# cfframe/spatial-VAE

Measured on AMD Instinct MI355X. Metric: images/sec (ELBO fwd+bwd+step), MNIST 28x28 batch=256, 1/2/4/8 GPU, higher is better.
Workload: dtype f32; 1 GPU; mnist-rotated-translated 28x28 z=2 H=500x2 tanh B=256 (BASELINE configs[1]); global_batch=256, per_gpu_batch=256, pixels=784, parallelism=dp1

## Files before the change

spatial_vae_amd/csrc/api.hip:

```cpp
#include <stdarg.h>
#include <stdio.h>
#include <stdlib.h>
#include <string.h>
#include <math.h>
#include <atomic>
#include <mutex>
#include <iterator>
#include <type_traits>
#include <unordered_map>
#include <vector>

#include "common.h"
#include <hip/hip_ext.h>
#include "dense.h"
#include "wgrad2.h"
#include "elementwise.h"
#include "encoder.h"
#include "split.h"

using namespace svae;

namespace {

thread_local char g_err[512] = "";
// ... 77 lines not shown
bool split_wgrad_on() {
    static const bool on = [] { const char* e = getenv("SVAE_SPLIT_WGRAD"); return !(e && e[0] == '0'); }();
    return on;
}

bool split_a0_fragments_only(const Geo& g) {
    static const bool on = [] { const char* e = getenv("SVAE_SPLIT_A0"); return e && e[0] == '1'; }();
    const char* fuse = getenv("SVAE_FUSE_OUT");
    return on && split_mode() && split_l0_on() && split_wgrad_on() && !(fuse && fuse[0] == '1') &&
           (g.act == SVAE_ACT_TANH || g.act == SVAE_ACT_SIGMOID) && g.ntile % 2 == 0 && g.L == 2 && g.in_dim == 2 &&
           !(g.flags & SVAE_FLAG_RESID);
}

int fuse_out_mode() {
    const char* e = getenv("SVAE_FUSE_OUT");
    if (!e) return 2;
    return e[0] == '0' ? 0 : (e[0] == '1' ? 1 : 2);
}
bool split_active(const Geo& g) {
    return split_mode() && (g.act == SVAE_ACT_TANH || g.act == SVAE_ACT_SIGMOID) && g.ntile % 2 == 0;
}
bool rank1_out(const Geo& g) {
    return fuse_out_mode() == 2 && !split_active(g) && g.C == 1 && g.L >= 2 && !(g.flags & SVAE_FLAG_RESID) &&
           (g.act == SVAE_ACT_TANH || g.act == SVAE_ACT_SIGMOID);
}

struct PlanBits {
    unsigned bits;
    unsigned long long seq;
};
std::mutex g_plan_mu;
std::unordered_map<const void*, PlanBits> g_plans;
unsigned long long g_plan_seq = 0;
unsigned plan_bits(const Geo& g) {
    return (rank1_out(g) ? 1u : 0u) | (split_active(g) ? 2u : 0u) | ((unsigned)fuse_out_mode() << 2) |
           (split_a0_fragments_only(g) ? 16u : 0u) | ((split_mode() && split_l0_on()) ? 32u : 0u);
}
void remember_plan(const void* saved, unsigned bits) {
    std::lock_guard<std::mutex> lk(g_plan_mu);
    if (g_plans.size() >= 4096) {
        const unsigned long long cut = g_plan_seq - 2048;
        for (auto it = g_plans.begin(); it != g_plans.end();) it = it->second.seq < cut ? g_plans.erase(it) : std::next(it);
    }
    g_plans[saved] = PlanBits{bits, g_plan_seq++};
}
long recorded_plan(const void* saved) {
    std::lock_guard<std::mutex> lk(g_plan_mu);
    auto it = g_plans.find(saved);
    return it == g_plans.end() ? -1L : (long)it->second.bits;
}

constexpr int kFinishMaxChunks = 64;
int finish_chunks(int N) {
    int c = (N + 1023) / 1024;
    return c < 1 ? 1 : (c > kFinishMaxChunks ? kFinishMaxChunks : c);
}

Plan make_plan(const Geo& g, void* saved, void* ws) {
    Plan p;
    const size_t MH = (size_t)g.Mp * g.Hp;
    Carver cs(saved);
    for (int l = 0; l < g.L; ++l) p.act[l] = cs.take<float>(MH);
    p.savedC = split_mode() ? cs.take<uint4>(MH / 4) : nullptr;
    float* swf[SVAE_MAX_HIDDEN];
    float* swb[SVAE_MAX_HIDDEN];
    for (int l = 0; l + 1 < g.L; ++l) {
        swf[l] = cs.take<float>((size_t)g.Hp * g.Hp);
        swb[l] = cs.take<float>((size_t)g.Hp * g.Hp);
    }
// ... 417 lines not shown
                               g.Hp, (const float*)pl.gscale);
        if (!aprev_cols)
            hipLaunchKernelGGL(split_cols_kernel, dim3(blocks_for(g.noct * g.Hp)), dim3(256), 0, st, aprev, pl.splitC[1],
                               g.noct, g.Hp, (const float*)nullptr);
    }
    Scope prof(K_WGRAD, st);
    static bool attr_set = false;
    if (!attr_set) {
        (void)hipFuncSetAttribute(reinterpret_cast<const void*>(&split_wgrad_kernel<true>),
                                  hipFuncAttributeMaxDynamicSharedMemorySize, kSplitWgradLds);
        (void)hipFuncSetAttribute(reinterpret_cast<const void*>(&split_wgrad_kernel<false>),
                                  hipFuncAttributeMaxDynamicSharedMemorySize, kSplitWgradLds);
        attr_set = true;
    }
    SplitWgradArgs w;
    w.dh = pl.splitC[0]; w.ap = aprev_cols ? aprev_cols : pl.splitC[1]; w.slab = pl.slab; w.bslab = pl.bslab; w.gscale = pl.gscale;
    w.nsteps = (long)g.Mp / 16; w.Hp = g.Hp; w.nblk1 = pl.wg_nblk1; w.S = pl.wg_S;
    const dim3 grid(pl.wg_nblk1 * pl.wg_nblk1 * pl.wg_S);
    if (cols_ready) hipLaunchKernelGGL(split_wgrad_kernel<false>, grid, dim3(256), kSplitWgradLds, st, w);
    else hipLaunchKernelGGL(split_wgrad_kernel<true>, grid, dim3(256), kSplitWgradLds, st, w);
}

int use_dense4(const Geo& g, int resid, int lastd) {
    const char* e = getenv("SVAE_DENSE4");
    const int mode = e ? (e[0] == '0' ? 0 : (e[0] == '2' ? 2 : 1)) : 3;
    if (mode == 0 || g.tiles % 4 != 0 || resid || lastd == 1) return 0;
    const bool nt2_ok = g.ntile % 2 == 0;
    if (mode == 2) return nt2_ok ? 2 : 1;
    if (mode == 1) return 1;
    const long wgs2 = ((g.tiles / 4 + 3) / 4) * (g.ntile / 2);
    return (nt2_ok && wgs2 >= 2048) ? 2 : 1;
}

template <int NT, bool DGRAD, bool FIRST, int LASTD, int CF>
void launch_dense4_v(const DenseArgs& a, long groups, long set0, long nsets, hipStream_t st) {
    const dim3 grid((unsigned)(((nsets + 7) / 8) * 8 * ((a.Hp / 32) / NT)));
    constexpr int lds = DenseCfg<NT>::LDS_BYTES + (FIRST ? 4 * 3 * 128 * 4 : 0);
    const long gend = (set0 + nsets) * 4 < groups ? (set0 + nsets) * 4 : groups;
    launch_gemm(dense4_kernel<NT, DGRAD, FIRST, LASTD, CF>, grid, dim3(256), (unsigned)lds, st, a, gend, set0);
}

struct DenseBlocks {
    int nt;
    long m_split;
    int nt_tail;
};

long dense4_main_sets(const Geo& g, long sets, bool tail_ok) {
    const char* e = getenv("SVAE_DENSE4_TAIL");
    if ((e && e[0] == '0') || !tail_ok) return sets;
    if (e && e[0] == '=') {
        const long k = atol(e + 1);
        return (k > 0 && k < sets) ? k : sets;
    }
    static const long slots = [] {
        int dev = 0, cus = 256;
        if (hipGetDevice(&dev) == hipSuccess) (void)hipDeviceGetAttribute(&cus, hipDeviceAttributeMultiprocessorCount, dev);
        return (long)cus * 2;
    }();
    const long nblk = g.ntile / 2;
    const long W = sets * nblk;
    if (slots % nblk != 0) return sets;
    const long full = (W / slots) * slots, rest = W - full;
    if (full < 2 * slots || rest == 0 || W >= 16 * slots || 20 * rest > 9 * slots) return sets;
    return full / nblk;
}

template <bool DGRAD, bool FIRST, int LASTD, int CF>
void launch_dense4_dual(const DenseArgs& a, long groups, long sets, long main_sets, hipStream_t st) {
    const unsigned ntile = (unsigned)(a.Hp / 32);
    const unsigned grid_main = (unsigned)(((main_sets + 7) / 8) * 8) * (ntile / 2);
    const unsigned grid_tail = (unsigned)(((sets - main_sets + 7) / 8) * 8) * ntile;
    constexpr int lds = DenseCfg<2>::LDS_BYTES + (FIRST ? 4 * 3 * 128 * 4 : 0);
    launch_gemm(dense4_dual_kernel<DGRAD, FIRST, LASTD, CF>, dim3(grid_main + grid_tail), dim3(256), (unsigned)lds, st, a, groups,
                main_sets, grid_main);
}

template <bool DGRAD>
DenseBlocks launch_dense(const Geo& g, const DenseArgs& a, hipStream_t st, bool first = false, int lastd = 0, int cf = 0) {
    took(DGRAD ? P_DENSE_FP32_DGRAD : P_DENSE_FP32_FWD);
    if (lastd) took(lastd == 1 ? P_OUT_BWD_FUSED_GENERIC : P_OUT_BWD_RANK1);
    Scope prof(DGRAD ? K_DENSE_DGRAD : K_DENSE_FWD, st, true);
    if (const int nt4 = use_dense4(g, a.resid, lastd)) {
        took(P_DENSE4);
        if (!DGRAD && cf > 0) took(P_DENSE4_CF);
        if (nt4 == 2) took(P_DENSE4_NT2);
        const long groups = g.tiles / 4;
        const long sets = (groups + 3) / 4;
        auto go = [&](auto nt_tag, long set0, long nsets) {
            constexpr int NT = decltype(nt_tag)::value;
            if constexpr (!DGRAD) {
                switch (cf) {
                    case 0: launch_dense4_v<NT, false, false, 0, 0>(a, groups, set0, nsets, st); break;
                    case 1: launch_dense4_v<NT, false, false, 0, 1>(a, groups, set0, nsets, st); break;
                    case 2: launch_dense4_v<NT, false, false, 0, 2>(a, groups, set0, nsets, st); break;
                    case 3: launch_dense4_v<NT, false, false, 0, 3>(a, groups, set0, nsets, st); break;
                    default: launch_dense4_v<NT, false, false, 0, 4>(a, groups, set0, nsets, st); break;
                }
            } else {
                if (first) {
                    if (lastd == 2) launch_dense4_v<NT, true, true, 2, 0>(a, groups, set0, nsets, st);
                    else if (lastd == 3) launch_dense4_v<NT, true, true, 3, 0>(a, groups, set0, nsets, st);
                    else launch_dense4_v<NT, true, true, 0, 0>(a, groups, set0, nsets, st);
                } else {
                    if (lastd == 2) launch_dense4_v<NT, true, false, 2, 0>(a, groups, set0, nsets, st);
                    else if (lastd == 3) launch_dense4_v<NT, true, false, 3, 0>(a, groups, set0, nsets, st);
                    else launch_dense4_v<NT, true, false, 0, 0>(a, groups, set0, nsets, st);
                }
            }
        };
        if (nt4 == 1) {
            go(std::integral_constant<int, 1>(), 0, sets);
            return DenseBlocks{1, (long)g.Mp, 1};
        }
        if (cf > 2) {
            if constexpr (!DGRAD) {
                if (cf == 3) launch_dense4_v<2, false, false, 0, 3>(a, groups, 0, sets, st);
                else launch_dense4_v<2, false, false, 0, 4>(a, groups, 0, sets, st);
            }
            return DenseBlocks{2, (long)g.Mp, 1};
        }
        const long main_sets = dense4_main_sets(g, sets, true);
        took(P_DENSE4_DUAL);
        if (main_sets < sets) took(P_DENSE4_TAIL);
        if constexpr (!DGRAD) {
            switch (cf) {
                case 0: launch_dense4_dual<false, false, 0, 0>(a, groups, sets, main_sets, st); break;
                case 1: launch_dense4_dual<false, false, 0, 1>(a, groups, sets, main_sets, st); break;
                default: launch_dense4_dual<false, false, 0, 2>(a, groups, sets, main_sets, st); break;
            }
        } else {
            if (first) {
                if (lastd == 2) launch_dense4_dual<true, true, 2, 0>(a, groups, sets, main_sets, st);
                else if (lastd == 3) launch_dense4_dual<true, true, 3, 0>(a, groups, sets, main_sets, st);
                else launch_dense4_dual<true, true, 0, 0>(a, groups, sets, main_sets, st);
            } else {
                if (lastd == 2) launch_dense4_dual<true, false, 2, 0>(a, groups, sets, main_sets, st);
                else if (lastd == 3) launch_dense4_dual<true, false, 3, 0>(a, groups, sets, main_sets, st);
                else launch_dense4_dual<true, false, 0, 0>(a, groups, sets, main_sets, st);
            }
        }
        return DenseBlocks{2, main_sets < sets ? main_sets * 512 : (long)g.Mp, 1};
    }
    const int nt = (first || lastd || cf) ? dense_nt_first(g.ntile) : dense_nt_for(g.ntile);
    static const bool xcd_grid = [] { const char* e = getenv("SVAE_XCD_GRID"); return !(e && e[0] == '0'); }();
    const long groups = (g.tiles + 3) / 4;
    const dim3 grid = (xcd_grid && g.ntile / nt > 1) ? dim3((unsigned)(((groups + 7) / 8) * 8 * (g.ntile / nt)))
                                                     : dim3((unsigned)groups, (unsigned)(g.ntile / nt));
    switch (nt) {
        case 16: launch_dense_nt<16, DGRAD>(a, grid, st, first, lastd, cf); break;
        case 8: launch_dense_nt<8, DGRAD>(a, grid, st, first, lastd, cf); break;
        case 4: launch_dense_nt<4, DGRAD>(a, grid, st, first, lastd, cf); break;
        case 2: launch_dense_nt<2, DGRAD>(a, grid, st, first, lastd, cf); break;
        default: launch_dense_nt<1, DGRAD>(a, grid, st, first, lastd, cf); break;
    }
    return DenseBlocks{nt, (long)g.Mp, nt};
}

template <int CL, int R1 = 0>
void launch_wgrad_c(const WgradArgs& w, dim3 grid, hipStream_t st) {
    static bool attr_set = false;
    if (!attr_set) {
        (void)hipFuncSetAttribute(reinterpret_cast<const void*>(&wgrad_kernel<CL, R1>), hipFuncAttributeMaxDynamicSharedMemorySize,
                                  kWgradLdsBytes);
        attr_set = true;
    }
    launch_gemm(wgrad_kernel<CL, R1>, grid, dim3(256), (unsigned)kWgradLdsBytes, st, w);
}

bool tail_merge_on() {
    const char* e = getenv("SVAE_TAIL_MERGE");
    return !(e && e[0] == '0');
}

bool use_wgrad2(int cl, int r1) {
// ... 39 lines not shown
template <int ACT>
void launch_layer0_fwd(const Geo& g, const Plan& pl, const PoseArgs& pa, float* a0, hipStream_t st) {
    Scope prof(K_LAYER0_FWD, st);
    const int oimg = g.Npad / 8;
    const int cpi = (oimg + kL0Chunk - 1) / kL0Chunk;
    const int opc = (oimg + cpi - 1) / cpi;
    const long nchunks = (long)g.B * cpi;
    const unsigned gy = (unsigned)(nchunks < 32768 ? nchunks : 32768);
    const unsigned gz = (unsigned)((nchunks + gy - 1) / gy);
    hipLaunchKernelGGL((layer0_fwd_kernel<ACT>), dim3(blocks_for(g.Hp * 2), gy, gz), dim3(256), 0, st, pa, pl.posebuf,
                       pl.tab, a0, row_geo(g), opc, (oimg + opc - 1) / opc, nchunks);
}

template <int ACT>
void launch_layer0_fwd_split(const Geo& g, const Plan& pl, const PoseArgs& pa, float* a0, bool saved_ok, hipStream_t st) {
    Scope prof(K_LAYER0_FWD, st);
    hipLaunchKernelGGL((layer0_fwd_split_kernel<ACT>), dim3((unsigned)g.tiles, (unsigned)(g.Hp / 64)), dim3(256), 0, st, pa,
                       pl.posebuf, pl.tab, split_a0_fragments_only(g) ? (float*)nullptr : a0, pl.splitA,
                       (saved_ok && g.L == 2) ? pl.savedC : (uint4*)nullptr, row_geo(g));
}

template <int C>
void launch_out_fwd(const Geo& g, const float* a, const svae_params* p, float* y, float* logits, hipStream_t st) {
    Scope prof(K_OUT_FWD, st);
    long nb = (g.noct + 3) / 4;
    if (nb > 4096) nb = 4096;
    hipLaunchKernelGGL((out_fwd_kernel<C>), dim3((unsigned)nb), dim3(256), 0, st, a, p->out_w, p->out_b, y, logits,
                       row_geo(g), g.H, (g.flags & SVAE_FLAG_SOFTPLUS) ? 1 : 0, g.noct);
}

template <int ACT, int C>
void launch_out_bwd_ac(const Geo& g, const Plan& pl, const float* a, const svae_params* p, float* dh, hipStream_t st) {
    Scope prof(K_OUT_BWD, st);
    hipLaunchKernelGGL((out_bwd_kernel<ACT, C>), dim3(blocks_for(g.Hp * 2), pl.ob_chunks), dim3(256), 0, st, a, pl.do_p,
                       p->out_w, dh, pl.wpart, pl.bpart, g.H, g.Hp, (long)g.Mp, g.noct, pl.ob_oct_per_chunk);
}
template <int ACT>
void launch_out_bwd_a(const Geo& g, const Plan& pl, const float* a, const svae_params* p, float* dh, hipStream_t st) {
    took(P_OUT_BWD_STREAM);
    switch (g.C) {
        case 1: launch_out_bwd_ac<ACT, 1>(g, pl, a, p, dh, st); break;
        case 2: launch_out_bwd_ac<ACT, 2>(g, pl, a, p, dh, st); break;
        case 3: launch_out_bwd_ac<ACT, 3>(g, pl, a, p, dh, st); break;
        default: launch_out_bwd_ac<ACT, 4>(g, pl, a, p, dh, st); break;
    }
}

}

extern "C" {

int svae_abi_version(void) { return SVAE_ABI_VERSION; }
const char* svae_last_error(void) { return g_err; }

size_t svae_saved_bytes(const svae_desc* d) {
    if (check_desc(d) != SVAE_OK) return 0;
    return make_plan(make_geo(*d), nullptr, nullptr).saved_bytes;
}

size_t svae_workspace_bytes(const svae_desc* d) {
    if (check_desc(d) != SVAE_OK) return 0;
    return make_plan(make_geo(*d), nullptr, nullptr).ws_bytes;
}

}

namespace {
int decoder_forward_impl(const svae_desc* d, const svae_params* p, const svae_pose* pose, const float* z, float* y,
// ... 99 lines not shown
}
}

extern "C" {

int svae_decoder_forward(const svae_desc* d, const svae_params* p, const svae_pose* pose, const float* z, float* y,
                         float* logits, void* saved, void* ws, size_t ws_bytes, svae_stream_t stream) {
    return decoder_forward_impl(d, p, pose, z, y, logits, saved, ws, ws_bytes, stream, nullptr, nullptr, nullptr);
}

int svae_decoder_forward_bce(const svae_desc* d, const svae_params* p, const svae_pose* pose, const float* z,
                             const float* target, float* y, float* logits, float* loglik, float* dll_dy, void* saved, void* ws,
                             size_t ws_bytes, svae_stream_t stream) {
    if (!target) return fail(SVAE_E_INVALID, "svae_decoder_forward_bce: target is null");
    return decoder_forward_impl(d, p, pose, z, y, logits, saved, ws, ws_bytes, stream, target, loglik, dll_dy);
}

int svae_decoder_backward(const svae_desc* d, const svae_params* p, const svae_pose* pose, const float* z,
                          const float* logits, const float* dy, const float* dy_scale, const void* saved,
                          const svae_grads* grads, float* dz, const svae_pose_grads* pg, void* ws, size_t ws_bytes,
                          svae_stream_t stream) {
    int rc;
    if ((rc = check_desc(d)) || (rc = check_params(d, p)) || (rc = check_pose(pose))) return rc;
    if (!logits || !dy || !saved || !grads) return fail(SVAE_E_INVALID, "logits, dy, saved and grads are required");
    if (d->Zd > 0 && !z) return fail(SVAE_E_INVALID, "latent_dim > 0 but z is null");
    if (reinterpret_cast<uintptr_t>(saved) & 255) return fail(SVAE_E_WORKSPACE, "saved not 256-byte aligned");
    if (pg && (pg->dtheta || pg->ddx) && pose->coords)
        return fail(SVAE_E_INVALID, "dtheta/ddx requested but the pose was given as explicit coords");
    const Geo g = make_geo(*d);
    {
        const long rec = recorded_plan(saved);
        if (rec >= 0 && (unsigned)rec != plan_bits(g))
            return fail(SVAE_E_INVALID, "svae_decoder_backward: `saved` was written by a forward call planned differently (plan "
                        "bits %ld then, %u now): the GEMM mode (svae_gemm_mode_set / SVAE_GEMM) or SVAE_FUSE_OUT changed between "
                        "the forward call and its backward call", rec, plan_bits(g));
    }
    const Plan pl = make_plan(g, const_cast<void*>(saved), ws);
    if ((rc = check_ws(pl, ws, ws_bytes))) return rc;
    hipStream_t st = static_cast<hipStream_t>(stream);
    const PoseArgs pa = pose_args(pose);
    const int resid = (g.flags & SVAE_FLAG_RESID) ? 1 : 0;
    const int fmode = fuse_out_mode();
    const bool split_bwd = split_active(g) && g.L >= 2 && fmode != 1;
    const bool r1 = rank1_out(g);

    {
        Scope prof(K_DLOGITS, st);
        if (split_bwd && hipMemsetAsync(pl.amax, 0, sizeof(unsigned), st) != hipSuccess) return fail(SVAE_E_LAUNCH, "memset failed");
        hipLaunchKernelGGL(dlogits_kernel, dim3(blocks_for((long)g.C * g.Mp)), dim3(256), 0, st, logits, dy, dy_scale,
                           pl.do_p, g.B, g.N, g.Npad, g.C, (g.flags & SVAE_FLAG_SOFTPLUS) ? 1 : 0, (long)g.Mp,
                           split_bwd ? pl.amax : (unsigned*)nullptr);
        if (split_bwd)
            hipLaunchKernelGGL(split_scale_kernel, dim3(1), dim3(256), 0, st, pl.amax, p->out_w, g.C, g.H, pl.gscale);
    }

    int cur = 0;
    const bool fused_out = r1 || (fmode == 1 && g.L >= 2 && !resid && (grads->hidden_w[g.L - 2] || grads->hidden_b[g.L - 2]));
    int ob_nparts = 0;
    static const bool ob_env = [] { const char* e = getenv("SVAE_SPLIT_OB"); return !(e && e[0] == '0'); }();
    const bool split_ob = ob_env && split_bwd && split_wgrad_on() && (grads->hidden_w[g.L - 2] || grads->hidden_b[g.L - 2]);
    if (split_ob) {
        const float* alast = pl.act[g.L - 1];
        float* dh32 = resid ? pl.dh[cur] : nullptr;
        const int nparts = g.act == SVAE_ACT_TANH ? launch_out_bwd_split_a<SVAE_ACT_TANH>(g, pl, alast, p, dh32, st)
                                                  : launch_out_bwd_split_a<SVAE_ACT_SIGMOID>(g, pl, alast, p, dh32, st);
        ob_nparts = nparts;
        Scope prof(K_SMALL_BWD, st);
        hipLaunchKernelGGL(out_bwd_reduce_kernel, dim3(g.C * ((g.Hp + 63) / 64) + 1), dim3(1024), 0, st, pl.wpart, pl.bpart,
// ... 406 lines not shown
```

spatial_vae_amd/csrc/dense.h:

```cpp
#pragma once
#include "common.h"

namespace svae {

struct DenseArgs {
    const float* in;
    const float* wp;
    float* out;
    const float* bias;
    const float* aux;
    long tiles;
    int Hp;
    int H;
    int act;
    int resid;
    PoseArgs pose;
    const float4* posebuf;
    const float* tab;
    float* sgtile;
    float* dfpart;
    long Mp;
    int N, Timg;
    const float* do_p;
    const float* out_w;
    int C;
    float* lpart;
};

template <int ACT, bool DGRAD>
__device__ __forceinline__ float4 dense_epilogue(float4 v, float bias, float4 aux) {
    if (DGRAD) {
        v.x *= act_grad<ACT>(aux.x); v.y *= act_grad<ACT>(aux.y);
        v.z *= act_grad<ACT>(aux.z); v.w *= act_grad<ACT>(aux.w);
    } else {
        v.x = act_fwd<ACT>(v.x + bias); v.y = act_fwd<ACT>(v.y + bias);
        v.z = act_fwd<ACT>(v.z + bias); v.w = act_fwd<ACT>(v.w + bias);
    }
    return v;
}

__device__ __forceinline__ void glds16(const float* gsrc, unsigned lds_byte_addr) {
    unsigned keep;
    asm volatile(
        "s_mov_b32 %0, m0\n\ts_mov_b32 m0, %2\n\ts_nop 0\n\tglobal_load_lds_dwordx4 %1, off\n\ts_mov_b32 m0, %0"
        : "=&s"(keep)
        : "v"(gsrc), "s"(lds_byte_addr)
        : "memory");
}
__device__ __forceinline__ void dma_wait_all() { asm volatile("s_waitcnt vmcnt(0)" ::: "memory"); }
__device__ __forceinline__ void glds16_s(const void* sbase, unsigned voff, unsigned lds_byte_addr) {
    unsigned keep;
    asm volatile(
        "s_mov_b32 %0, m0\n\ts_mov_b32 m0, %3\n\ts_nop 0\n\tglobal_load_lds_dwordx4 %1, %2\n\ts_mov_b32 m0, %0"
        : "=&s"(keep)
        : "v"(voff), "s"(sbase), "s"(lds_byte_addr)
        : "memory");
}

__device__ __forceinline__ void load_a_chunk(const float* p, float (&v)[4][4]) {
// ... 739 lines not shown
```

spatial_vae_amd/csrc/dense4.h:

```cpp
#pragma once
#include "dense.h"

namespace svae {

typedef float f32x4v __attribute__((ext_vector_type(4)));
typedef float f32x2v __attribute__((ext_vector_type(2)));

template <int OFF>
__device__ __forceinline__ void load_a4(const float* p, f32x4v& v) {
    asm volatile("global_load_dwordx4 %0, %1, off offset:%2" : "+v"(v) : "v"(p), "i"(OFF) : "memory");
}
template <int N>
__device__ __forceinline__ void wait_vm4(f32x4v& v) {
    asm volatile("s_waitcnt vmcnt(%1)" : "+v"(v) : "i"(N) : "memory");
}
template <int LASTD>
__device__ __forceinline__ f32x4v rank1_actgrad(f32x4v x) {
    f32x4v r;
#pragma unroll
    for (int i = 0; i < 4; ++i) r[i] = __builtin_fmaf(-x[i], x[i], LASTD == 2 ? 1.0f : x[i]);
    return r;
}

template <int NT>
struct Dense4Occ {
    static constexpr int value = NT == 1 ? 3 : 2;
};

template <int NT, bool DGRAD, bool FIRST, int LASTD, int CF>
__device__ __forceinline__ void dense4_body(const DenseArgs& a, long groups, long set0, unsigned bid) {
    static_assert(NT == 1 || NT == 2, "4 NT accumulator tiles: two waves per SIMD up to NT = 2");
    static_assert(!FIRST || DGRAD, "FIRST is a data-gradient epilogue");
    static_assert(LASTD == 0 || ((LASTD == 2 || LASTD == 3) && DGRAD), "LASTD: the rank-1 data-gradient forms only");
    static_assert(CF == 0 || (!DGRAD && CF <= SVAE_MAX_OUT), "CF = output channels of the forward epilogue's W_o contraction");
    extern __shared__ __attribute__((aligned(16))) float smem[];
    using Cfg = DenseCfg<NT>;
    constexpr int NB = Cfg::NB, G = Cfg::G, CHUNK = Cfg::CHUNK, NINSTR = Cfg::NINSTR;
    const int lane = threadIdx.x & 63;
    const int wave = __builtin_amdgcn_readfirstlane(threadIdx.x >> 6);
    const int nl = lane & 31, h = lane >> 5;
    const int Hp = a.Hp;
    const int noct = Hp / 8;
    const int nchunk = noct / G;
    const int ntile = Hp / 32;
    const int nblk = ntile / NT;
    const long local = bid >> 3;
    const int nb = (int)(local % nblk);
    const long set = set0 + (local / nblk) * 8 + (bid & 7);
    const long rg = set * 4 + wave;
    const bool live = rg < groups;
    const long rgl = live ? rg : groups - 1;

    const float* arow = a.in + ((rgl * 16 + (nl >> 1)) * (long)Hp + 4 * h) * 8 + (nl & 1) * 4;
    const float* bfrag = smem + lane * 4;
    const unsigned lds_base = (unsigned)(size_t)(__attribute__((address_space(3))) float*)smem;

    f32x16 acc[4][NT];
#pragma unroll
    for (int c = 0; c < 4; ++c)
#pragma unroll
        for (int t = 0; t < NT; ++t)
#pragma unroll
            for (int r = 0; r < 16; ++r) acc[c][t][r] = 0.0f;

    constexpr int PW = (NINSTR + 3) / 4;
    unsigned poff[PW], pm0[PW];
#pragma unroll
    for (int j = 0; j < PW; ++j) {
        const int idx = wave + 4 * j;
        const int gl = (idx < NINSTR ? idx : NINSTR - 1) / NT, tt = (idx < NINSTR ? idx : NINSTR - 1) % NT;
        poff[j] = (unsigned)(((gl * ntile + nb * NT + tt) * 256 + lane * 4) * 4);
        pm0[j] = lds_base + (unsigned)(idx < NINSTR ? idx : NINSTR - 1) * 1024u;
    }
    const unsigned chunk_bytes = (unsigned)(G * ntile) * 1024u;
    auto stage_piece = [&](int c, int buf, int j) {
        glds16_s(reinterpret_cast<const char*>(a.wp) + (long)c * chunk_bytes, poff[j], pm0[j] + (unsigned)(buf * CHUNK) * 4u);
    };
    auto stage = [&](int c, int buf) {
#pragma unroll
        for (int j = 0; j < PW; ++j) stage_piece(c, buf, j);
    };
    auto read_b = [&](int o, float4 (&b)[NT]) {
        const float* base = bfrag + ((o / G) & 1) * CHUNK + (o % G) * NT * 256;
#pragma unroll
        for (int t = 0; t < NT; ++t) b[t] = *reinterpret_cast<const float4*>(base + t * 256);
    };
    constexpr int P = PW;
    constexpr int PE = (P + 3) / 4;
    static_assert(G == 4, "the slot offsets assume 4 octets per chunk");

    float* rowx = smem + 2 * CHUNK + wave * (3 * 128);
    if (FIRST) {
#pragma unroll
        for (int rr = 0; rr < 2; ++rr) {
            const int row = lane + 64 * rr;
            const long tile = rgl * 4 + (row >> 5);
            const int b = (int)(tile / a.Timg);
            const int i = (int)(tile % a.Timg) * 32 + (row & 31);
            const float4 pb = a.posebuf[b];
            const float* cbase = a.pose.coords ? a.pose.coords + (long)b * a.N * 2 : a.pose.grid;
            const float2 g2 = *reinterpret_cast<const float2*>(cbase + (long)(i < a.N ? i : a.N - 1) * 2);
            const bool in = i < a.N;
            rowx[row] = in ? pb.x * g2.x - pb.y * g2.y + pb.z : 0.0f;
            rowx[128 + row] = in ? pb.y * g2.x + pb.x * g2.y + pb.w : 0.0f;
            if (LASTD != 0) rowx[256 + row] = a.do_p[rgl * 128 + row];
        }
    }
    stage(0, 0);
    stage(nchunk > 1 ? 1 : 0, 1);
    f32x4v av[G][4];
    float4 b0[NT], b1[NT];
#pragma unroll
    for (int gl = 0; gl < G; ++gl)
#pragma unroll
        for (int e = 0; e < 4; ++e) av[gl][e] = f32x4v{0.0f, 0.0f, 0.0f, 0.0f};
    load_a4<0>(arow, av[0][0]); load_a4<32>(arow, av[0][1]); load_a4<64>(arow, av[0][2]); load_a4<96>(arow, av[0][3]);
    load_a4<256>(arow, av[1][0]); load_a4<288>(arow, av[1][1]); load_a4<320>(arow, av[1][2]); load_a4<352>(arow, av[1][3]);
    load_a4<512>(arow, av[2][0]); load_a4<544>(arow, av[2][1]); load_a4<576>(arow, av[2][2]); load_a4<608>(arow, av[2][3]);
    load_a4<768>(arow, av[3][0]); load_a4<800>(arow, av[3][1]); load_a4<832>(arow, av[3][2]); load_a4<864>(arow, av[3][3]);
#pragma unroll
    for (int gl = 0; gl < G; ++gl)
#pragma unroll
        for (int e = 0; e < 4; ++e) wait_vm4<0>(av[gl][e]);
    __syncthreads();
    read_b(0, b0);
    const int spare = nchunk & 1;
    auto kstep = [&](const f32x4v& x, const float4 (&bf)[NT], int e) {
#pragma unroll
        for (int t = 0; t < NT; ++t) {
            const float bv = e == 0 ? bf[t].x : e == 1 ? bf[t].y : e == 2 ? bf[t].z : bf[t].w;
            acc[0][t] = __builtin_amdgcn_mfma_f32_32x32x2f32(x[0], bv, acc[0][t], 0, 0, 0);
            acc[1][t] = __builtin_amdgcn_mfma_f32_32x32x2f32(x[1], bv, acc[1][t], 0, 0, 0);
            acc[2][t] = __builtin_amdgcn_mfma_f32_32x32x2f32(x[2], bv, acc[2][t], 0, 0, 0);
            acc[3][t] = __builtin_amdgcn_mfma_f32_32x32x2f32(x[3], bv, acc[3][t], 0, 0, 0);
        }
    };
    auto reload = [&](int gl, int e, const float* anext) {
        if (gl == 0 && e == 0) load_a4<0>(anext, av[0][0]);
// ... 36 lines not shown
                reload(gl, e, anext);
                if (gl == G - 1) {
#pragma unroll
                    for (int j = 0; j < PE; ++j)
                        if (e * PE + j < P) stage_piece(cstage, bstage, e * PE + j);
                }
                __builtin_amdgcn_sched_barrier(0);
            }
        }
    }
    {
#pragma unroll
        for (int gl = 0; gl < G; ++gl)
#pragma unroll
            for (int e = 0; e < 4; ++e) wait_vm4<0>(av[gl][e]);
        const int o0 = (nchunk - 1) * G;
        const int gtail = (a.H + 7) / 8 - o0;
#pragma unroll
        for (int gl = 0; gl < G; ++gl) {
            if (gl < gtail) {
                if (gl + 1 < G) { if (gl & 1) read_b(o0 + gl + 1, b0); else read_b(o0 + gl + 1, b1); }
#pragma unroll
                for (int e = 0; e < 4; ++e) {
                    const f32x4v x = LASTD != 0 ? rank1_actgrad<LASTD>(av[gl][e]) : av[gl][e];
                    if (LASTD != 0) __builtin_amdgcn_sched_barrier(0);
                    if (gl & 1) kstep(x, b1, e); else kstep(x, b0, e);
                    if (LASTD != 0) __builtin_amdgcn_sched_barrier(0);
                }
            }
        }
    }
    if (!live) return;

    auto epi = [&](auto act_tag) {
        constexpr int ACT = decltype(act_tag)::value;
        constexpr int NS = 4 * NT;
        float bias[NT];
#pragma unroll
        for (int t = 0; t < NT; ++t) {
            const int n = nb * NB + t * 32 + nl;
            const float bv = DGRAD ? 0.0f : a.bias[n < a.H ? n : a.H - 1];
            bias[t] = (n < a.H) ? bv : 0.0f;
        }
        auto voff = [&](int q, int r, int t) -> long {
            return ((rgl * 16 + 4 * q + 2 * h + (r >> 1)) * (long)Hp + nb * NB + t * 32 + nl) * 8 + 4 * (r & 1);
        };
        auto value = [&](int q, int r, int t, const float4& aux, const float4& dq) -> float4 {
            float4 v = make_float4(acc[0][t][4 * q + r], acc[1][t][4 * q + r], acc[2][t][4 * q + r], acc[3][t][4 * q + r]);
            v = dense_epilogue<ACT, DGRAD>(v, bias[t], aux);
            if (LASTD != 0) { v.x *= dq.x; v.y *= dq.y; v.z *= dq.z; v.w *= dq.w; }
            return v;
        };
        if (!FIRST) {
            float4 xa[2][4];
            float4 dqv[2][4];
            auto fetch_aux = [&](int s_, float4 (&fa)[4]) {
                const int q = s_ / NT, t = s_ % NT;
#pragma unroll
                for (int r = 0; r < 4; ++r) fa[r] = *reinterpret_cast<const float4*>(a.aux + voff(q, r, t));
            };
            auto fetch_dq = [&](int q, float4 (&d)[4]) {
#pragma unroll
                for (int r = 0; r < 4; ++r) d[r] = *reinterpret_cast<const float4*>(a.do_p + rgl * 128 + 32 * q + 16 * h + 4 * r);
            };
            constexpr int CFN = CF > 0 ? CF : 1;
            float wo[CFN][NT], lp[CFN][16];
            if (CF > 0) {
#pragma unroll
                for (int c = 0; c < CFN; ++c)
#pragma unroll
                    for (int t = 0; t < NT; ++t) {
                        const int n = nb * NB + t * 32 + nl;
                        const float wv = a.out_w[c * a.H + (n < a.H ? n : a.H - 1)];
                        wo[c][t] = (n < a.H) ? wv : 0.0f;
                    }
            }
            if (DGRAD) fetch_aux(0, xa[0]);
            if (LASTD != 0) fetch_dq(0, dqv[0]);
#pragma unroll
            for (int s_ = 0; s_ < NS; ++s_) {
                const int q = s_ / NT, t = s_ % NT;
                if (s_ + 1 < NS) {
                    if (DGRAD) fetch_aux(s_ + 1, xa[(s_ + 1) & 1]);
                    if (LASTD != 0 && (s_ + 1) % NT == 0) fetch_dq((s_ + 1) / NT, dqv[((s_ + 1) / NT) & 1]);
                }
                if (CF > 0 && t == 0) {
#pragma unroll
                    for (int c = 0; c < CFN; ++c)
#pragma unroll
                        for (int j = 0; j < 16; ++j) lp[c][j] = 0.0f;
                }
#pragma unroll
                for (int r = 0; r < 4; ++r) {
                    const float4 v = value(q, r, t, xa[s_ & 1][r], dqv[q & 1][r]);
                    *reinterpret_cast<float4*>(a.out + voff(q, r, t)) = v;
                    if (CF > 0) {
#pragma unroll
                        for (int c = 0; c < CFN; ++c) {
                            lp[c][4 * r] += v.x * wo[c][t]; lp[c][4 * r + 1] += v.y * wo[c][t];
                            lp[c][4 * r + 2] += v.z * wo[c][t]; lp[c][4 * r + 3] += v.w * wo[c][t];
                        }
                    }
                }
                if (CF > 0 && t == NT - 1) {
#pragma unroll
                    for (int c = 0; c < CFN; ++c) {
                        float s4[4];
                        half_reduce16(lp[c], s4);
                        if (nl < 4) {
                            const int cls = ((nl & 1) << 1) | (nl >> 1);
                            *reinterpret_cast<float4*>(a.lpart + ((long)nb * CFN + c) * a.Mp + rgl * 128 + 32 * q + 16 * h + 4 * cls) =
                                make_float4(s4[0], s4[1], s4[2], s4[3]);
                        }
                    }
                }
            }
        } else {
            float4 xa[2][NT][2];
            auto fetch_aux = [&](int hp, float4 (&fa)[NT][2]) {
                const int q = hp >> 1, rh = hp & 1;
#pragma unroll
                for (int t = 0; t < NT; ++t)
#pragma unroll
                    for (int r2 = 0; r2 < 2; ++r2) fa[t][r2] = *reinterpret_cast<const float4*>(a.aux + voff(q, 2 * rh + r2, t));
            };
            fetch_aux(0, xa[0]);
            float2 w[NT];
            float sv[NT], g0[NT], g1[NT];
#pragma unroll
            for (int hp = 0; hp < 8; ++hp) {
                const int q = hp >> 1, rh = hp & 1;
                const long tile = rgl * 4 + q;
                if (rh == 0) {
                    const int b = (int)(tile / a.Timg);
#pragma unroll
                    for (int t = 0; t < NT; ++t) {
                        w[t] = *reinterpret_cast<const float2*>(a.tab + ((long)b * Hp + nb * NB + t * 32 + nl) * kSlots);
                        sv[t] = 0.0f; g0[t] = 0.0f; g1[t] = 0.0f;
                    }
                }
                if (hp + 1 < 8) fetch_aux(hp + 1, xa[(hp + 1) & 1]);
                const float* rx = rowx + 32 * q + 16 * h + 8 * rh;
                float4 x0v[2], x1v[2], dq[2];
#pragma unroll
                for (int r2 = 0; r2 < 2; ++r2) {
                    x0v[r2] = *reinterpret_cast<const float4*>(rx + 4 * r2);
                    x1v[r2] = *reinterpret_cast<const float4*>(rx + 128 + 4 * r2);
                    if (LASTD != 0) dq[r2] = *reinterpret_cast<const float4*>(rx + 256 + 4 * r2);
                }
                float pd[16];
#pragma unroll
                for (int j = 0; j < 16; ++j) pd[j] = 0.0f;
#pragma unroll
                for (int t = 0; t < NT; ++t)
#pragma unroll
                    for (int r2 = 0; r2 < 2; ++r2) {
                        const float4 v = value(q, 2 * rh + r2, t, xa[hp & 1][t][r2], dq[r2]);
                        const float vv[4] = {v.x, v.y, v.z, v.w};
                        const float xx0[4] = {x0v[r2].x, x0v[r2].y, x0v[r2].z, x0v[r2].w};
                        const float xx1[4] = {x1v[r2].x, x1v[r2].y, x1v[r2].z, x1v[r2].w};
#pragma unroll
                        for (int cc = 0; cc < 4; ++cc) {
                            const int j = 4 * r2 + cc;
                            sv[t] += vv[cc];
                            g0[t] += vv[cc] * xx0[cc];
                            g1[t] += vv[cc] * xx1[cc];
                            pd[j] += vv[cc] * w[t].x;
                            pd[8 + j] += vv[cc] * w[t].y;
                        }
                    }
                float s4[4];
                half_reduce16(pd, s4);
                if (nl < 4) {
                    const int cls = ((nl & 1) << 1) | (nl >> 1);
                    float* dst = a.dfpart + ((long)nb * a.Mp + tile * 32 + 16 * h + 8 * rh + 4 * (cls & 1)) * 2 + (cls >> 1);
                    dst[0] = s4[0]; dst[2] = s4[1]; dst[4] = s4[2]; dst[6] = s4[3];
                }
                if (rh == 1) {
#pragma unroll
                    for (int t = 0; t < NT; ++t) {
                        const float G0 = g0[t] + __shfl_xor(g0[t], 32), G1 = g1[t] + __shfl_xor(g1[t], 32);
                        const float S = sv[t] + __shfl_xor(sv[t], 32);
                        const int k = nb * NB + t * 32 + nl;
                        if (h == 0) *reinterpret_cast<float4*>(a.sgtile + (tile * (long)Hp + k) * 4) = make_float4(G0, G1, S, 0.0f);
                    }
                }
            }
        }
    };
    switch (a.act) {
        case SVAE_ACT_TANH: epi(std::integral_constant<int, SVAE_ACT_TANH>()); break;
        case SVAE_ACT_LEAKYRELU: epi(std::integral_constant<int, SVAE_ACT_LEAKYRELU>()); break;
        case SVAE_ACT_RELU: epi(std::integral_constant<int, SVAE_ACT_RELU>()); break;
        default: epi(std::integral_constant<int, SVAE_ACT_SIGMOID>()); break;
    }
}

template <int NT, bool DGRAD, bool FIRST, int LASTD, int CF>
__global__ __launch_bounds__(256, Dense4Occ<NT>::value) void dense4_kernel(DenseArgs a, long groups, long set0) {
    dense4_body<NT, DGRAD, FIRST, LASTD, CF>(a, groups, set0, blockIdx.x);
}

template <bool DGRAD, bool FIRST, int LASTD, int CF>
__global__ __launch_bounds__(256, 2) void dense4_dual_kernel(DenseArgs a, long groups, long sets_main, unsigned grid_main) {
    if (blockIdx.x < grid_main) {
        const long gmain = sets_main * 4 < groups ? sets_main * 4 : groups;
        dense4_body<2, DGRAD, FIRST, LASTD, CF>(a, gmain, 0, blockIdx.x);
    } else {
        dense4_body<1, DGRAD, FIRST, LASTD, CF>(a, groups, sets_main, blockIdx.x - grid_main);
    }
}

}
```

spatial_vae_amd/csrc/elementwise.h:

```cpp
#pragma once
#include <type_traits>
#include "common.h"

namespace svae {

__device__ __forceinline__ long slab_index(int contr, int out, int ntile) {
    return (((long)(contr >> 3) * ntile + (out >> 5)) * 2 + ((contr >> 2) & 1)) * 128 + (out & 31) * 4 + (contr & 3);
}
struct PrepareArgs {
    const float* coord_w; const float* coord_b; const float* latent_w; const float* bil_w; const float* z;
    float* tab; float4* posebuf; PoseArgs pose;
    int B, H, Hp, Zd, in_dim;
    int nb_tab, nb_pack, nlayers;
    const float* W[SVAE_MAX_HIDDEN]; float* wf[SVAE_MAX_HIDDEN]; float* wb[SVAE_MAX_HIDDEN];
    const float* wb_row_scale[SVAE_MAX_HIDDEN];
};
__global__ void __launch_bounds__(256) prepare_kernel(PrepareArgs a) {
    if ((int)blockIdx.x < a.nb_tab) {
        const long idx = (long)blockIdx.x * 256 + threadIdx.x;
        if (idx < a.B) {
            float c, s, d0, d1;
            image_pose(a.pose, (int)idx, c, s, d0, d1);
            a.posebuf[idx] = make_float4(c, s, d0, d1);
        }
// ... 195 lines not shown
    if (idx < (long)C * Mp) {
        const int c = (int)(idx / Mp);
        const long mp = idx - (long)c * Mp;
        const int b = (int)(mp / Npad), i = (int)(mp - (long)b * Npad);
        float v = 0.0f;
        if (i < N) {
            const long src = ((long)b * N + i) * C + c;
            const float lg = logits[src];
            const float s = 1.0f / (1.0f + expf(-lg));
            float g = dy[src];
            if (dy_scale) g *= dy_scale[b];
            if (softplus && c == 0) g *= 1.0f / (1.0f + expf(-s));
            v = g * s * (1.0f - s);
        }
        do_p[idx] = v;
        m = fabsf(v);
    }
    if (amax) {
        __shared__ float red[4];
#pragma unroll
        for (int d = 32; d >= 1; d >>= 1) m = fmaxf(m, __shfl_xor(m, d));
        if ((threadIdx.x & 63) == 0) red[threadIdx.x >> 6] = m;
        __syncthreads();
        if (threadIdx.x == 0) {
            m = fmaxf(fmaxf(red[0], red[1]), fmaxf(red[2], red[3]));
            if (m > 0.0f) atomicMax(amax, __float_as_uint(m));
        }
    }
}

template <int ACT, int C>
__global__ void out_bwd_kernel(const float* __restrict__ a, const float* __restrict__ do_p,
                               const float* __restrict__ out_w, float* __restrict__ dh, float* __restrict__ wpart,
                               float* __restrict__ bpart, int H, int Hp, long Mp, long noct, long oct_per_chunk) {
    const int t = blockIdx.x * 256 + threadIdx.x;
    if (t >= Hp * 2) return;
    const int h = t & 1, n = t >> 1;
    float w[C], pw[C], pb[C];
#pragma unroll
    for (int c = 0; c < C; ++c) {
        w[c] = (n < H) ? out_w[c * H + n] : 0.0f;
        pw[c] = 0.0f;
        pb[c] = 0.0f;
    }
    const long o0 = blockIdx.y * oct_per_chunk;
    const long o1 = (o0 + oct_per_chunk < noct) ? o0 + oct_per_chunk : noct;
    for (long o = o0; o < o1; ++o) {
        const long off = (o * Hp + n) * 8 + 4 * h;
        const float4 av = *reinterpret_cast<const float4*>(a + off);
        float4 da = make_float4(0.f, 0.f, 0.f, 0.f);
#pragma unroll
        for (int c = 0; c < C; ++c) {
            const float4 d = *reinterpret_cast<const float4*>(do_p + (long)c * Mp + 8 * o + 4 * h);
            da.x += d.x * w[c]; da.y += d.y * w[c]; da.z += d.z * w[c]; da.w += d.w * w[c];
            pw[c] += (d.x * av.x + d.y * av.y) + (d.z * av.z + d.w * av.w);
            pb[c] += (d.x + d.y) + (d.z + d.w);
        }
        da.x *= act_grad<ACT>(av.x); da.y *= act_grad<ACT>(av.y);
        da.z *= act_grad<ACT>(av.z); da.w *= act_grad<ACT>(av.w);
        *reinterpret_cast<float4*>(dh + off) = da;
    }
#pragma unroll
    for (int c = 0; c < C; ++c) wpart[(((long)blockIdx.y * 2 + h) * C + c) * Hp + n] = pw[c];
    if (n == 0) {
#pragma unroll
        for (int c = 0; c < C; ++c) bpart[((long)blockIdx.y * 2 + h) * C + c] = pb[c];
    }
}

constexpr int kObrLanes = 16;
__global__ void __launch_bounds__(1024) out_bwd_reduce_kernel(const float* __restrict__ wpart, const float* __restrict__ bpart,
                                                              float* __restrict__ dWo, float* __restrict__ dbo, int C, int H,
                                                              int Hp, int nparts) {
    __shared__ float red[kObrLanes][65];
    const int col = threadIdx.x & 63, pl = threadIdx.x >> 6;
    const int blocks_per_c = (Hp + 63) / 64;
    if (blockIdx.x == (unsigned)(C * blocks_per_c)) {
        float s = 0.0f;
        if (col < C)
            for (int i = pl; i < nparts; i += kObrLanes) s += bpart[(long)i * C + col];
// ... 821 lines not shown
```

Before: 96180 images/s.

## Compact padded rows in dense4 GEMMs to skip per-image padding tiles

When the pixel count N is a multiple of 16 but not 32 (e.g. 784), the dense4 forward and dgrad kernels now iterate over a compacted row space of B*N rows instead of the padded B*Npad rows. Row, image and tile-slot indices are remapped, with special handling for half-tiles that straddle an image boundary. out_bwd also skips padded octets. This is meant to remove the wasted GEMM work on padding rows (784 padded to 800), at the cost of extra integer index arithmetic and more complex epilogue addressing.

```diff
diff --git a/spatial_vae_amd/csrc/api.hip b/spatial_vae_amd/csrc/api.hip
--- a/spatial_vae_amd/csrc/api.hip
+++ b/spatial_vae_amd/csrc/api.hip
@@ -133,9 +133,11 @@
 std::mutex g_plan_mu;
 std::unordered_map<const void*, PlanBits> g_plans;
 unsigned long long g_plan_seq = 0;
+int compact_hpi(const Geo& g);
 unsigned plan_bits(const Geo& g) {
     return (rank1_out(g) ? 1u : 0u) | (split_active(g) ? 2u : 0u) | ((unsigned)fuse_out_mode() << 2) |
-           (split_a0_fragments_only(g) ? 16u : 0u) | ((split_mode() && split_l0_on()) ? 32u : 0u);
+           (split_a0_fragments_only(g) ? 16u : 0u) | ((split_mode() && split_l0_on()) ? 32u : 0u) |
+           (compact_hpi(g) ? 64u : 0u);
 }
 void remember_plan(const void* saved, unsigned bits) {
     std::lock_guard<std::mutex> lk(g_plan_mu);
@@ -619,6 +621,15 @@
     return (nt2_ok && wgs2 >= 2048) ? 2 : 1;
 }
 
+int compact_hpi(const Geo& g) {
+    const char* e = getenv("SVAE_COMPACT_ROWS");
+    if (e && e[0] == '0') return 0;
+    if (g.N % 16 != 0 || g.N % 32 == 0 || ((long)g.B * g.N) % 128 != 0) return 0;
+    if ((g.flags & SVAE_FLAG_RESID) || fuse_out_mode() == 1 || split_mode()) return 0;
+    if (!use_dense4(g, 0, 0)) return 0;
+    return g.N / 16;
+}
+
 template <int NT, bool DGRAD, bool FIRST, int LASTD, int CF>
 void launch_dense4_v(const DenseArgs& a, long groups, long set0, long nsets, hipStream_t st) {
     const dim3 grid((unsigned)(((nsets + 7) / 8) * 8 * ((a.Hp / 32) / NT)));
@@ -664,7 +675,9 @@
 }
 
 template <bool DGRAD>
-DenseBlocks launch_dense(const Geo& g, const DenseArgs& a, hipStream_t st, bool first = false, int lastd = 0, int cf = 0) {
+DenseBlocks launch_dense(const Geo& g, const DenseArgs& args, hipStream_t st, bool first = false, int lastd = 0, int cf = 0) {
+    DenseArgs a = args;
+    a.hpi = 0;
     took(DGRAD ? P_DENSE_FP32_DGRAD : P_DENSE_FP32_FWD);
     if (lastd) took(lastd == 1 ? P_OUT_BWD_FUSED_GENERIC : P_OUT_BWD_RANK1);
     Scope prof(DGRAD ? K_DENSE_DGRAD : K_DENSE_FWD, st, true);
@@ -672,8 +685,10 @@
         took(P_DENSE4);
         if (!DGRAD && cf > 0) took(P_DENSE4_CF);
         if (nt4 == 2) took(P_DENSE4_NT2);
-        const long groups = g.tiles / 4;
+        a.hpi = compact_hpi(g);
+        const long groups = a.hpi ? (long)g.B * g.N / 128 : g.tiles / 4;
         const long sets = (groups + 3) / 4;
+        auto actual_row = [&](long m) { return a.hpi ? (m / g.N) * g.Npad + m % g.N : m; };
         auto go = [&](auto nt_tag, long set0, long nsets) {
             constexpr int NT = decltype(nt_tag)::value;
             if constexpr (!DGRAD) {
@@ -727,7 +742,7 @@
                 else launch_dense4_dual<true, false, 0, 0>(a, groups, sets, main_sets, st);
             }
         }
-        return DenseBlocks{2, main_sets < sets ? main_sets * 512 : (long)g.Mp, 1};
+        return DenseBlocks{2, main_sets < sets ? actual_row(main_sets * 512) : (long)g.Mp, 1};
     }
     const int nt = (first || lastd || cf) ? dense_nt_first(g.ntile) : dense_nt_for(g.ntile);
     static const bool xcd_grid = [] { const char* e = getenv("SVAE_XCD_GRID"); return !(e && e[0] == '0'); }();
@@ -833,8 +848,9 @@
 template <int ACT, int C>
 void launch_out_bwd_ac(const Geo& g, const Plan& pl, const float* a, const svae_params* p, float* dh, hipStream_t st) {
     Scope prof(K_OUT_BWD, st);
+    const int po = g.Npad / 8, vo = compact_hpi(g) ? g.N / 8 : po;
     hipLaunchKernelGGL((out_bwd_kernel<ACT, C>), dim3(blocks_for(g.Hp * 2), pl.ob_chunks), dim3(256), 0, st, a, pl.do_p,
-                       p->out_w, dh, pl.wpart, pl.bpart, g.H, g.Hp, (long)g.Mp, g.noct, pl.ob_oct_per_chunk);
+                       p->out_w, dh, pl.wpart, pl.bpart, g.H, g.Hp, (long)g.Mp, g.noct, pl.ob_oct_per_chunk, vo, po);
 }
 template <int ACT>
 void launch_out_bwd_a(const Geo& g, const Plan& pl, const float* a, const svae_params* p, float* dh, hipStream_t st) {
@@ -1000,8 +1016,8 @@
         const long rec = recorded_plan(saved);
         if (rec >= 0 && (unsigned)rec != plan_bits(g))
             return fail(SVAE_E_INVALID, "svae_decoder_backward: `saved` was written by a forward call planned differently (plan "
-                        "bits %ld then, %u now): the GEMM mode (svae_gemm_mode_set / SVAE_GEMM) or SVAE_FUSE_OUT changed between "
-                        "the forward call and its backward call", rec, plan_bits(g));
+                        "bits %ld then, %u now): the GEMM mode (svae_gemm_mode_set / SVAE_GEMM), SVAE_FUSE_OUT, SVAE_DENSE4 or "
+                        "SVAE_COMPACT_ROWS changed between the forward call and its backward call", rec, plan_bits(g));
     }
     const Plan pl = make_plan(g, const_cast<void*>(saved), ws);
     if ((rc = check_ws(pl, ws, ws_bytes))) return rc;
diff --git a/spatial_vae_amd/csrc/dense.h b/spatial_vae_amd/csrc/dense.h
--- a/spatial_vae_amd/csrc/dense.h
+++ b/spatial_vae_amd/csrc/dense.h
@@ -25,6 +25,7 @@
     const float* out_w;
     int C;
     float* lpart;
+    int hpi;
 };
 
 template <int ACT, bool DGRAD>
diff --git a/spatial_vae_amd/csrc/dense4.h b/spatial_vae_amd/csrc/dense4.h
--- a/spatial_vae_amd/csrc/dense4.h
+++ b/spatial_vae_amd/csrc/dense4.h
@@ -47,11 +47,22 @@
     const long local = bid >> 3;
     const int nb = (int)(local % nblk);
     const long set = set0 + (local / nblk) * 8 + (bid & 7);
+    if (set * 4 >= groups) return;
     const long rg = set * 4 + wave;
     const bool live = rg < groups;
     const long rgl = live ? rg : groups - 1;
-
-    const float* arow = a.in + ((rgl * 16 + (nl >> 1)) * (long)Hp + 4 * h) * 8 + (nl & 1) * 4;
+    const int hpi = a.hpi;
+    const int Npad = a.Timg * 32;
+
+    const float* arow;
+    if (hpi) {
+        const unsigned cq = (unsigned)rgl * 32u + (unsigned)nl;
+        const unsigned b = cq / (unsigned)(4 * hpi);
+        const unsigned row = b * (unsigned)Npad + 4u * (cq - b * (unsigned)(4 * hpi));
+        arow = a.in + ((long)(row >> 3) * Hp + 4 * h) * 8 + (row & 4u);
+    } else {
+        arow = a.in + ((rgl * 16 + (nl >> 1)) * (long)Hp + 4 * h) * 8 + (nl & 1) * 4;
+    }
     const float* bfrag = smem + lane * 4;
     const unsigned lds_base = (unsigned)(size_t)(__attribute__((address_space(3))) float*)smem;
 
@@ -94,16 +105,23 @@
 #pragma unroll
         for (int rr = 0; rr < 2; ++rr) {
             const int row = lane + 64 * rr;
-            const long tile = rgl * 4 + (row >> 5);
-            const int b = (int)(tile / a.Timg);
-            const int i = (int)(tile % a.Timg) * 32 + (row & 31);
+            int b, i;
+            if (hpi) {
+                const unsigned cr = (unsigned)rgl * 128u + (unsigned)row;
+                b = (int)(cr / (unsigned)a.N);
+                i = (int)(cr - (unsigned)b * (unsigned)a.N);
+            } else {
+                const long tile = rgl * 4 + (row >> 5);
+                b = (int)(tile / a.Timg);
+                i = (int)(tile % a.Timg) * 32 + (row & 31);
+            }
             const float4 pb = a.posebuf[b];
             const float* cbase = a.pose.coords ? a.pose.coords + (long)b * a.N * 2 : a.pose.grid;
             const float2 g2 = *reinterpret_cast<const float2*>(cbase + (long)(i < a.N ? i : a.N - 1) * 2);
             const bool in = i < a.N;
             rowx[row] = in ? pb.x * g2.x - pb.y * g2.y + pb.z : 0.0f;
             rowx[128 + row] = in ? pb.y * g2.x + pb.x * g2.y + pb.w : 0.0f;
-            if (LASTD != 0) rowx[256 + row] = a.do_p[rgl * 128 + row];
+            if (LASTD != 0) rowx[256 + row] = a.do_p[(long)b * Npad + i];
         }
     }
     stage(0, 0);
@@ -206,6 +224,37 @@
     }
     if (!live) return;
 
+    int ub[4] = {0, 0, 0, 0}, uj[4] = {0, 0, 0, 0};
+    if (hpi) {
+        const unsigned ht = (unsigned)rg * 8u;
+        unsigned b = ht / (unsigned)hpi, j = ht - b * (unsigned)hpi;
+#pragma unroll
+        for (int q = 0; q < 4; ++q) {
+            ub[q] = (int)b;
+            uj[q] = (int)j;
+            j += 2;
+            if (j >= (unsigned)hpi) { j -= (unsigned)hpi; ++b; }
+        }
+    }
+    auto half_at = [&](int q, int& row, int& img, int& slot) {
+        if (hpi) {
+            const bool wrap = uj[q] + h == hpi;
+            const int j = wrap ? 0 : uj[q] + h;
+            img = ub[q] + (wrap ? 1 : 0);
+            row = img * Npad + 16 * j;
+            slot = img * a.Timg + ((j + (img & 1)) >> 1);
+        } else {
+            row = (int)(rg * 128) + 32 * q + 16 * h;
+            img = FIRST ? (int)((rg * 4 + q) / a.Timg) : 0;
+            slot = (int)(rg * 4) + q;
+        }
+    };
+    auto half_row = [&](int q) {
+        int row, img, slot;
+        half_at(q, row, img, slot);
+        return row;
+    };
+
     auto epi = [&](auto act_tag) {
         constexpr int ACT = decltype(act_tag)::value;
         constexpr int NS = 4 * NT;
@@ -217,7 +266,7 @@
             bias[t] = (n < a.H) ? bv : 0.0f;
         }
         auto voff = [&](int q, int r, int t) -> long {
-            return ((rgl * 16 + 4 * q + 2 * h + (r >> 1)) * (long)Hp + nb * NB + t * 32 + nl) * 8 + 4 * (r & 1);
+            return (((long)(half_row(q) >> 3) + (r >> 1)) * Hp + nb * NB + t * 32 + nl) * 8 + 4 * (r & 1);
         };
         auto value = [&](int q, int r, int t, const float4& aux, const float4& dq) -> float4 {
             float4 v = make_float4(acc[0][t][4 * q + r], acc[1][t][4 * q + r], acc[2][t][4 * q + r], acc[3][t][4 * q + r]);
@@ -235,7 +284,7 @@
             };
             auto fetch_dq = [&](int q, float4 (&d)[4]) {
 #pragma unroll
-                for (int r = 0; r < 4; ++r) d[r] = *reinterpret_cast<const float4*>(a.do_p + rgl * 128 + 32 * q + 16 * h + 4 * r);
+                for (int r = 0; r < 4; ++r) d[r] = *reinterpret_cast<const float4*>(a.do_p + half_row(q) + 4 * r);
             };
             constexpr int CFN = CF > 0 ? CF : 1;
             float wo[CFN][NT], lp[CFN][16];
@@ -283,7 +332,7 @@
                         half_reduce16(lp[c], s4);
                         if (nl < 4) {
                             const int cls = ((nl & 1) << 1) | (nl >> 1);
-                            *reinterpret_cast<float4*>(a.lpart + ((long)nb * CFN + c) * a.Mp + rgl * 128 + 32 * q + 16 * h + 4 * cls) =
+                            *reinterpret_cast<float4*>(a.lpart + ((long)nb * CFN + c) * a.Mp + half_row(q) + 4 * cls) =
                                 make_float4(s4[0], s4[1], s4[2], s4[3]);
                         }
                     }
@@ -304,9 +353,10 @@
 #pragma unroll
             for (int hp = 0; hp < 8; ++hp) {
                 const int q = hp >> 1, rh = hp & 1;
-                const long tile = rgl * 4 + q;
+                int hrow, himg, hslot;
+                half_at(q, hrow, himg, hslot);
                 if (rh == 0) {
-                    const int b = (int)(tile / a.Timg);
+                    const int b = himg;
 #pragma unroll
                     for (int t = 0; t < NT; ++t) {
                         w[t] = *reinterpret_cast<const float2*>(a.tab + ((long)b * Hp + nb * NB + t * 32 + nl) * kSlots);
@@ -347,16 +397,19 @@
                 half_reduce16(pd, s4);
                 if (nl < 4) {
                     const int cls = ((nl & 1) << 1) | (nl >> 1);
-                    float* dst = a.dfpart + ((long)nb * a.Mp + tile * 32 + 16 * h + 8 * rh + 4 * (cls & 1)) * 2 + (cls >> 1);
+                    float* dst = a.dfpart + ((long)nb * a.Mp + hrow + 8 * rh + 4 * (cls & 1)) * 2 + (cls >> 1);
                     dst[0] = s4[0]; dst[2] = s4[1]; dst[4] = s4[2]; dst[6] = s4[3];
                 }
                 if (rh == 1) {
+                    const bool lone = hpi != 0 && uj[q] + 1 == hpi;
 #pragma unroll
                     for (int t = 0; t < NT; ++t) {
-                        const float G0 = g0[t] + __shfl_xor(g0[t], 32), G1 = g1[t] + __shfl_xor(g1[t], 32);
-                        const float S = sv[t] + __shfl_xor(sv[t], 32);
+                        const float o0 = __shfl_xor(g0[t], 32), o1 = __shfl_xor(g1[t], 32), os = __shfl_xor(sv[t], 32);
+                        const float G0 = lone ? g0[t] : g0[t] + o0, G1 = lone ? g1[t] : g1[t] + o1;
+                        const float S = lone ? sv[t] : sv[t] + os;
                         const int k = nb * NB + t * 32 + nl;
-                        if (h == 0) *reinterpret_cast<float4*>(a.sgtile + (tile * (long)Hp + k) * 4) = make_float4(G0, G1, S, 0.0f);
+                        if (h == 0 || lone)
+                            *reinterpret_cast<float4*>(a.sgtile + ((long)hslot * Hp + k) * 4) = make_float4(G0, G1, S, 0.0f);
                     }
                 }
             }
diff --git a/spatial_vae_amd/csrc/elementwise.h b/spatial_vae_amd/csrc/elementwise.h
--- a/spatial_vae_amd/csrc/elementwise.h
+++ b/spatial_vae_amd/csrc/elementwise.h
@@ -251,7 +251,8 @@
 template <int ACT, int C>
 __global__ void out_bwd_kernel(const float* __restrict__ a, const float* __restrict__ do_p,
                                const float* __restrict__ out_w, float* __restrict__ dh, float* __restrict__ wpart,
-                               float* __restrict__ bpart, int H, int Hp, long Mp, long noct, long oct_per_chunk) {
+                               float* __restrict__ bpart, int H, int Hp, long Mp, long noct, long oct_per_chunk, int vo,
+                               int po) {
     const int t = blockIdx.x * 256 + threadIdx.x;
     if (t >= Hp * 2) return;
     const int h = t & 1, n = t >> 1;
@@ -264,7 +265,9 @@
     }
     const long o0 = blockIdx.y * oct_per_chunk;
     const long o1 = (o0 + oct_per_chunk < noct) ? o0 + oct_per_chunk : noct;
-    for (long o = o0; o < o1; ++o) {
+    int oi = (int)(o0 % po);
+    for (long o = o0; o < o1; ++o, oi = oi + 1 == po ? 0 : oi + 1) {
+        if (oi >= vo) continue;
         const long off = (o * Hp + n) * 8 + 4 * h;
         const float4 av = *reinterpret_cast<const float4*>(a + off);
         float4 da = make_float4(0.f, 0.f, 0.f, 0.f);
```

Result: no change. 96700 images/s, median of 6 (+0.5%).
